# hongsukchoi/Pose2Mesh_RELEASE

Hardware: AMD Instinct MI355X
Metric: SMPL meshes/sec fwd+bwd at batch 256 (higher is better)
Workload: dtype f32 (emulated on the BF16 matrix pipe: every operand as 3 exact bf16 slices = 24-bit significands, 6 slice products per fp32 product, fp32 accumulate)

## Files before the change

### pose2mesh_release_amd/csrc/gemm.hip

```cpp
#include <cstdlib>
#include <type_traits>

#include "p2m_split.h"

namespace p2m {

constexpr int BM = 128;
constexpr int BK = 32;
constexpr int AS_LD = BK + 1;

struct GemmArgs {
  const float* A[3];
  const float* Bm;
  const float* bias;
  const float* addend;
  const float* act_scale;
  const float* act_shift;
  int act_relu;
  int pair_out;
  float* C[3];
  float* stats;
  long M;
  int nplanesA, Ka, a0_shift;
  int N, Nc;
// ... 359 lines not shown
    for (int ps = 0; ps < APASS; ps++) {
      int lf, lc;
      if (ROWS) {
        int i = rs_i0 + ps * AROWS + a_row;
        if (i >= g.nset) i = g.nset - 1;
        lf = g.ids[i];
        lc = g.compact ? i : lf;
      } else {
        long rf = m0 + ps * AROWS + a_row;
        if (rf >= g.M) rf = g.M - 1;
        lf = (int)(rf - m0);
        lc = lf;
      }
      voff0[ps] = (unsigned)(((lf >> g.a0_shift) * g.Ka + a_k4) * 4);
      voff12[ps] = (unsigned)((lc * g.Ka + a_k4) * 4);
    }
    const int b_nl = (pt >> 1) & 7;
    const int b_n = ((((pt % (BN * 2)) >> 1) >> 3) << 3) | ((b_nl & 3) << 1) | (b_nl >> 2), b_half = (pt & 1) * 8;
    const unsigned bx_voff = (unsigned)((((n0 + b_n) * 16) + b_half) * 2);
    const long bx_slice = (long)g.Npad * 16;

    f32x4 ra[NST][APASS];
    u32x4 rb[NST][NS];
    auto load_chunk = [&](int kc, f32x4 (&a)[APASS], u32x4 (&b)[NS]) {
      const int p = kc / cpp;
      const int k0 = (kc - p * cpp) * KB;
      const char* Ab = reinterpret_cast<const char*>(g.A[p] + (p == 0 ? sbase0 : sbase12) + k0);
#pragma unroll
      for (int ps = 0; ps < APASS; ps++)
#ifdef P2M_PL_ABL_NOLOAD
        a[ps] = f32x4{__uint_as_float(voff0[ps]), 1.f, 2.f, (float)(long)Ab};
#else
        a[ps] = *reinterpret_cast<const f32x4*>(Ab + (p == 0 ? voff0[ps] : voff12[ps]));
#endif
      const char* src0 = reinterpret_cast<const char*>(g.Bx + (long)((p * g.Ka + k0) >> 4) * (NS * bx_slice));
#pragma unroll
      for (int sl = 0; sl < NS; sl++) b[sl] = *reinterpret_cast<const u32x4*>(src0 + sl * 2 * bx_slice + bx_voff);
    };
    auto store_chunk = [&](int kc, f32x4 (&a)[APASS], const u32x4 (&b)[NS]) {
      const int buf = kc % NBUF;
      unsigned short* as = As + buf * A_BUF;
#pragma unroll
      for (int ps = 0; ps < APASS; ps++) asm volatile("" : "+v"(a[ps]));
      if (in_act && kc < cpp) {
        const f32x4 sc = *reinterpret_cast<const f32x4*>(&actco[kc * KB + a_k4]);
        const f32x4 sh = *reinterpret_cast<const f32x4*>(&actco[256 + kc * KB + a_k4]);
#pragma unroll
        for (int ps = 0; ps < APASS; ps++)
#pragma unroll
          for (int e = 0; e < 4; e++) a[ps][e] = fmaxf(fmaf(a[ps][e], sc[e], sh[e]), 0.f);
      }
#pragma unroll
      for (int ps = 0; ps < APASS; ps++) {
        u32x2 sl[NS];
#ifdef P2M_PL_ABL_NOSLICE
        for (int q = 0; q < NS; q++) sl[q] = u32x2{__float_as_uint(a[ps][q & 1]), __float_as_uint(a[ps][2 + (q & 1)])};
#else
        split_pack4<NS>(a[ps][0], a[ps][1], a[ps][2], a[ps][3], a_sc, sl);
#endif
        unsigned short* d = as + (ps * AROWS + a_row) * LDX + a_k4;
#pragma unroll
        for (int q = 0; q < NS; q++) *reinterpret_cast<u32x2*>(d + q * BM * LDX) = sl[q];
      }
      unsigned short* d = Bs + buf * B_BUF + b_n * LDX + b_half;
#pragma unroll
      for (int q = 0; q < NS; q++) *reinterpret_cast<u32x4*>(d + q * BN * LDX) = b[q];
    };
    const int last = n - 1;
#pragma unroll
    for (int i = 0; i < NST; i++) load_chunk(i < last ? i : last, ra[i], rb[i]);
#pragma unroll
    for (int i = 0; i < AHEAD; i++) {
      if (i < n) store_chunk(i, ra[i], rb[i]);
      load_chunk(NST + i < last ? NST + i : last, ra[i], rb[i]);
    }
    lds_barrier();
    int kc = 0;
    for (; kc + (NST - 1) + AHEAD + NST < n; kc += NST) {
#pragma unroll
      for (int i = 0; i < NST; i++) {
        store_chunk(kc + i + AHEAD, ra[(i + AHEAD) % NST], rb[(i + AHEAD) % NST]);
        load_chunk(kc + i + AHEAD + NST, ra[(i + AHEAD) % NST], rb[(i + AHEAD) % NST]);
        lds_barrier();
      }
    }
    for (; kc < n; kc += NST) {
#pragma unroll
      for (int i = 0; i < NST; i++) {
        if (kc + i < n) {
          if (kc + i + AHEAD < n) store_chunk(kc + i + AHEAD, ra[(i + AHEAD) % NST], rb[(i + AHEAD) % NST]);
          if (kc + i + AHEAD + NST < n) load_chunk(kc + i + AHEAD + NST, ra[(i + AHEAD) % NST], rb[(i + AHEAD) % NST]);
          lds_barrier();
        }
      }
    }
  } else {
    frag_t fa[NBUF - 1][NS][TM], fb[NBUF - 1][NS][TN];
    auto read_frags = [&](int kc, frag_t (&a)[NS][TM], frag_t (&b)[NS][TN]) {
      const int buf = kc % NBUF;
      const unsigned short* as = As + buf * A_BUF + (wm * 64 + l31) * LDX + lhi * 8;
      const unsigned short* bs = Bs + buf * B_BUF + (wn * WTN + l31) * LDX + lhi * 8;
#pragma unroll
      for (int sl = 0; sl < NS; sl++) {
#pragma unroll
        for (int i = 0; i < TM; i++)
          a[sl][i] = __builtin_bit_cast(frag_t, *reinterpret_cast<const u32x4*>(as + (sl * BM + i * 32) * LDX));
#pragma unroll
        for (int j = 0; j < TN; j++)
          b[sl][j] = __builtin_bit_cast(frag_t, *reinterpret_cast<const u32x4*>(bs + (sl * BN + j * 32) * LDX));
      }
    };
    auto mfmas = [&](const frag_t (&a)[NS][TM], const frag_t (&b)[NS][TN]) {
#define P2M_PAIR(SA, SB)                                                                       \
  _Pragma("unroll") for (int i = 0; i < TM; i++) _Pragma("unroll") for (int j = 0; j < TN; j++) \
      acc[i][j] = slice_mfma<NS>(a[SA][i], b[SB][j], acc[i][j]);
#ifdef P2M_PL_ABL_NOMFMA
      if constexpr (NS == 3) {
        P2M_PAIR(0, 0)
        for (int sl = 1; sl < NS; sl++)
          for (int i = 0; i < TM; i++) for (int j = 0; j < TN; j++) { asm volatile("" :: "v"(a[sl][i])); asm volatile("" :: "v"(b[sl][j])); }
      } else
#endif
      if constexpr (NS == 3) {
        P2M_PAIR(2, 0)
        P2M_PAIR(0, 2)
        P2M_PAIR(1, 1)
        P2M_PAIR(1, 0)
        P2M_PAIR(0, 1)
        P2M_PAIR(0, 0)
      } else {
        P2M_PAIR(1, 0)
        P2M_PAIR(0, 1)
        P2M_PAIR(0, 0)
      }
#undef P2M_PAIR
    };
    lds_barrier();
    for (int kc = 0; kc < n; kc++) {
      read_frags(kc, fa[0], fb[0]);
      mfmas(fa[0], fb[0]);
      lds_barrier();
    }
  }
  __syncthreads();
  if (!producer) {
    gemm_epilogue<BN, EXTRA, ROWS>(g, acc, smem, rowtab, mt, m0, n0, rs_i0, wm, wn, l31, lhi, descale);
  } else {
    if (g.stats != nullptr) {
      __syncthreads();
      __syncthreads();
      __syncthreads();
    }
  }
}

template <int NS>
__global__ void k_weight_split(const float* __restrict__ Bm, unsigned short* __restrict__ Bx, int K, int N, int Npad,
                               const unsigned* __restrict__ amax_in, int bits) {
  const long i = (long)blockIdx.x * blockDim.x + threadIdx.x;
  if (i >= (long)Npad * K) return;
  const int k = (int)(i / Npad), n = (int)(i - (long)k * Npad);
  const long sl = (long)Npad * 16;
  unsigned short* d = Bx + (long)(k >> 4) * NS * sl + (long)n * 16 + (k & 15);
  if constexpr (NS == 3) {
    unsigned h = 0, m = 0, l = 0;
    if (n < N) split3(Bm[(long)k * N + n], h, m, l);
    d[0] = (unsigned short)(h >> 16);
    d[sl] = (unsigned short)(m >> 16);
    d[2 * sl] = (unsigned short)(l >> 16);
  } else {
    unsigned* trailer = reinterpret_cast<unsigned*>(Bx + (long)NS * Npad * K);
    const unsigned word = *amax_in;
    if (i == 0 && amax_in != trailer) *trailer = word == 0u ? 0u : __float_as_uint(__builtin_ldexpf(__uint_as_float(word), bits));
    const float y = n < N ? Bm[(long)k * N + n] * exp2_int(slice_scale_exp(word, bits)) : 0.f;
    const _Float16 h = (_Float16)y;
    const _Float16 l = (_Float16)(y - (float)h);
    d[0] = __builtin_bit_cast(unsigned short, h);
    d[sl] = __builtin_bit_cast(unsigned short, l);
  }
}

__global__ __launch_bounds__(1024) void k_amax_one_block(const float* __restrict__ x, long n, unsigned* __restrict__ word) {
  __shared__ float red[16];
  float m = 0.f;
  const long n4 = (reinterpret_cast<uintptr_t>(x) & 15) == 0 ? n >> 2 : 0;
  const f32x4* x4 = reinterpret_cast<const f32x4*>(x);
  long i = threadIdx.x;
  for (; i + 7 * 1024 < n4; i += 8 * 1024) {
    f32x4 v[8];
#pragma unroll
    for (int u = 0; u < 8; u++) v[u] = x4[i + u * 1024];
#pragma unroll
    for (int u = 0; u < 8; u++)
      m = fmaxf(fmaxf(m, fmaxf(amax_abs(v[u][0]), amax_abs(v[u][1]))), fmaxf(amax_abs(v[u][2]), amax_abs(v[u][3])));
  }
  for (; i < n4; i += 1024) {
    const f32x4 v = x4[i];
    m = fmaxf(fmaxf(m, fmaxf(amax_abs(v[0]), amax_abs(v[1]))), fmaxf(amax_abs(v[2]), amax_abs(v[3])));
  }
  for (long j = n4 * 4 + threadIdx.x; j < n; j += 1024) m = fmaxf(m, amax_abs(x[j]));
#pragma unroll
  for (int o = 32; o > 0; o >>= 1) m = fmaxf(m, __shfl_xor(m, o));
  if ((threadIdx.x & 63) == 0) red[threadIdx.x >> 6] = m;
  __syncthreads();
  if (threadIdx.x == 0) {
    for (int w = 1; w < 16; w++) m = fmaxf(m, red[w]);
    *word = __float_as_uint(m);
  }
}
__device__ __forceinline__ void amax_commit_block(unsigned* word, float m) {
  __shared__ float wmax[4];
#pragma unroll
  for (int o = 32; o > 0; o >>= 1) m = fmaxf(m, __shfl_xor(m, o));
  if ((threadIdx.x & 63) == 0) wmax[threadIdx.x >> 6] = m;
  __syncthreads();
  if (threadIdx.x == 0) {
    m = fmaxf(fmaxf(wmax[0], wmax[1]), fmaxf(wmax[2], wmax[3]));
    if (m > 0.f) {
      const unsigned bits = __float_as_uint(m);
      if (bits > __hip_atomic_load(word, __ATOMIC_RELAXED, __HIP_MEMORY_SCOPE_AGENT)) atomicMax(word, bits);
    }
  }
}
__global__ __launch_bounds__(256) void k_amax(const float* __restrict__ x, int head, long n4, int tail,
                                              unsigned* __restrict__ word) {
  float m = 0.f;
  const f32x4* x4 = reinterpret_cast<const f32x4*>(x + head);
  const long stride = (long)gridDim.x * 256;
  long i = (long)blockIdx.x * 256 + threadIdx.x;
  for (; i + 3 * stride < n4; i += 4 * stride) {
    const f32x4 v0 = x4[i], v1 = x4[i + stride], v2 = x4[i + 2 * stride], v3 = x4[i + 3 * stride];
    auto mx = [](const f32x4& v) {
      return fmaxf(fmaxf(amax_abs(v[0]), amax_abs(v[1])), fmaxf(amax_abs(v[2]), amax_abs(v[3])));
    };
    m = fmaxf(m, fmaxf(fmaxf(mx(v0), mx(v1)), fmaxf(mx(v2), mx(v3))));
  }
  for (; i < n4; i += stride) {
    const f32x4 v = x4[i];
    m = fmaxf(fmaxf(m, fmaxf(amax_abs(v[0]), amax_abs(v[1]))), fmaxf(amax_abs(v[2]), amax_abs(v[3])));
  }
  if (blockIdx.x == 0) {
    if ((int)threadIdx.x < head) m = fmaxf(m, amax_abs(x[threadIdx.x]));
    if ((int)threadIdx.x < tail) m = fmaxf(m, amax_abs(x[head + n4 * 4 + threadIdx.x]));
  }
  amax_commit_block(word, m);
}
__global__ __launch_bounds__(256) void k_amax_rows(const float* __restrict__ x, RowSet rs, int B, int F,
                                                   unsigned* __restrict__ word) {
  const int f4 = F >> 2;
  const long tot = (long)B * rs.n * f4;
  float m = 0.f;
  for (long i = (long)blockIdx.x * 256 + threadIdx.x; i < tot; i += (long)gridDim.x * 256) {
    const long row = i / f4;
    const int c = (int)(i - row * f4);
    const int b = (int)(row / rs.n), r = (int)(row - (long)b * rs.n);
    const f32x4 v = *reinterpret_cast<const f32x4*>(x + ((long)b * rs.V + (rs.ids ? rs.ids[r] : r)) * F + c * 4);
    m = fmaxf(fmaxf(m, fmaxf(amax_abs(v[0]), amax_abs(v[1]))), fmaxf(amax_abs(v[2]), amax_abs(v[3])));
  }
  amax_commit_block(word, m);
}

__global__ void k_naive_gemm_planes(GemmArgs g) {
  long idx = (long)blockIdx.x * blockDim.x + threadIdx.x;
  if (idx >= g.M * g.N) return;
  long r = idx / g.N;
  int n = (int)(idx - r * g.N);
  float acc = 0.f;
  for (int p = 0; p < g.nplanesA; p++) {
    const float* a = g.A[p] + (r >> (p == 0 ? g.a0_shift : 0)) * g.Ka;
    const float* b = g.Bm + (long)p * g.Ka * g.N + n;
    for (int k = 0; k < g.Ka; k++) acc = fmaf(a[k], b[(long)k * g.N], acc);
  }
  if (g.bias) acc += g.bias[n];
  if (g.act_scale) acc = fmaf(acc, g.act_scale[n], g.act_shift[n]);
  if (g.act_relu) acc = fmaxf(acc, 0.f);
  if (g.addend) acc += g.addend[r * g.N + n];
  int q = n / g.Nc;
  g.C[q][r * g.Nc + (n - q * g.Nc)] = acc;
}

__global__ void k_naive_tile_stats(const float* __restrict__ Y, float* __restrict__ stats, long M, int N) {
  int tile = blockIdx.x;
  long r0 = (long)tile * BM;
  long r1 = r0 + BM < M ? r0 + BM : M;
  for (int n = threadIdx.x; n < N; n += blockDim.x) {
    float s = 0.f;
    for (long r = r0; r < r1; r++) s += Y[r * N + n];
    float mean = s / (float)(r1 - r0);
    float m2 = 0.f;
    for (long r = r0; r < r1; r++) {
      float d = Y[r * N + n] - mean;
      m2 += d * d;
    }
    stats[(long)tile * 2 * N + n] = s;
    stats[(long)tile * 2 * N + N + n] = m2;
  }
}

struct TnArgs {
  const float* A[3];
  const float* G[3];
  int Gc;
  float* P;
  float* Pdb;
  long M, chunk_rows;
  int nplanesA, Ka, a0_shift, Ktot, N;
// ... 677 lines not shown
      k = (int)(kk / Fin); fin = (int)(kk % Fin);
    } else if (layout == 2) {
      fout = (int)(idx / Fin);
      fin = (int)(idx - (long)fout * Fin);
    } else {
      long nn = idx % ((long)K * Fout);
      fin = (int)(idx / ((long)K * Fout));
      k = (int)(nn / Fout); fout = (int)(nn % Fout);
    }
    float t0 = 0.f, t1 = 0.f, t2 = 0.f, t3 = 0.f;
    int c = cg;
    for (; c + 3 * UNP_CG < nchunks; c += 4 * UNP_CG) {
      t0 += P[(long)c * tot + idx];
      t1 += P[(long)(c + UNP_CG) * tot + idx];
      t2 += P[(long)(c + 2 * UNP_CG) * tot + idx];
      t3 += P[(long)(c + 3 * UNP_CG) * tot + idx];
    }
    for (; c < nchunks; c += UNP_CG) t0 += P[(long)c * tot + idx];
    s = ((double)t0 + (double)t1) + ((double)t2 + (double)t3);
    if (P2 != nullptr) {
      const long o2 = (long)fin * Fout + fout, st2 = (long)Fin * Fout;
      float q0 = 0.f, q1 = 0.f;
      int c2 = cg;
      for (; c2 + UNP_CG < nchunks2; c2 += 2 * UNP_CG) {
        q0 += P2[(long)c2 * st2 + o2];
        q1 += P2[(long)(c2 + UNP_CG) * st2 + o2];
      }
      for (; c2 < nchunks2; c2 += UNP_CG) q0 += P2[(long)c2 * st2 + o2];
      s += ((double)q0 + (double)q1) * (k == 0 ? 1.0 : (k == 1 ? (double)fake_a : (double)fake_b));
    }
  }
  red[cg][e] = s;
  __syncthreads();
  if (cg == 0 && idx < tot) {
    double r = 0.0;
#pragma unroll
    for (int q = 0; q < UNP_CG; q++) r += red[q][e];
    const long o = (long)fout * Fin * K + (long)fin * K + k;
    dW[o] = accumulate ? dW[o] + (float)r : (float)r;
  }
  if (db != nullptr && Pdb != nullptr && (long)blockIdx.x * 32 < Fout) {
    __syncthreads();
    double r = 0.0;
    if (idx < Fout) {
      for (int c = cg; c < nchunks; c += UNP_CG) r += (double)Pdb[(long)c * pdb_stride + idx];
      if (Pdb2 != nullptr)
        for (int c2 = cg; c2 < nchunks2; c2 += UNP_CG) r += (double)Pdb2[(long)c2 * Fout + idx];
    }
    red[cg][e] = r;
    __syncthreads();
    if (cg == 0 && idx < Fout) {
      double t = 0.0;
#pragma unroll
      for (int q = 0; q < UNP_CG; q++) t += red[q][e];
      db[idx] = accumulate ? db[idx] + (float)t : (float)t;
    }
  }
}

}

using namespace p2m;

extern "C" int32_t p2m_stats_tile_rows(void) { return BM; }


static inline int slices_of(int arith) { return arith == P2M_ARITH_F16X2 ? 2 : 3; }
static inline const unsigned* weight_amax_word(const void* Bx, int arith, long Npad, long K) {
  return arith == P2M_ARITH_F16X2
             ? reinterpret_cast<const unsigned*>(static_cast<const unsigned short*>(Bx) + 2 * Npad * K)
             : nullptr;
}

extern "C" int64_t p2m_weight_split_elems(int32_t K, int32_t N, int32_t arith) {
  if (K <= 0 || N <= 0 || K % 16 != 0 || (arith != P2M_ARITH_BF16X3 && arith != P2M_ARITH_F16X2)) return 0;
  return (long)slices_of(arith) * (cdiv(N, 128) * 128ll) * K + (arith == P2M_ARITH_F16X2 ? 8 : 0);
}

extern "C" int p2m_weight_split(const float* Bm, int32_t K, int32_t N, int32_t arith, const void* amax_in,
                                int32_t amax_bits, void* Bx, void* stream) {
  P2M_CHECK_ARG(Bm && Bx && K > 0 && N > 0, "null pointer or empty shape");
  P2M_CHECK_ARG(K % 16 == 0, "K must be a multiple of 16");
  P2M_CHECK_ARG(arith == P2M_ARITH_BF16X3 || arith == P2M_ARITH_F16X2, "arith must be P2M_ARITH_BF16X3 or P2M_ARITH_F16X2");
  const int Npad = cdiv(N, 128) * 128;
  const dim3 grid(cdiv((long)Npad * K, 256));
  unsigned short* bx = static_cast<unsigned short*>(Bx);
  if (arith == P2M_ARITH_F16X2) {
    const unsigned* word = static_cast<const unsigned*>(amax_in);
    P2M_CHECK_ARG(amax_bits >= 0 && amax_bits <= 30, "amax_bits out of range");
    if (word == nullptr) {
      unsigned* trailer = const_cast<unsigned*>(weight_amax_word(Bx, arith, Npad, K));
      hipLaunchKernelGGL(k_amax_one_block, dim3(1), dim3(1024), 0, (hipStream_t)stream, Bm, (long)K * N, trailer);
      word = trailer;
      amax_bits = 0;
    }
    hipLaunchKernelGGL(k_weight_split<2>, grid, dim3(256), 0, (hipStream_t)stream, Bm, bx, K, N, Npad, word, amax_bits);
  } else {
    hipLaunchKernelGGL(k_weight_split<3>, grid, dim3(256), 0, (hipStream_t)stream, Bm, bx, K, N, Npad, nullptr, 0);
  }
  return check_launch("weight_split");
}

extern "C" int p2m_conv_weights_prepare(const p2m_conv_weights* dev_desc, int32_t n, int32_t arith, void* stream) {
  static_assert(sizeof(p2m_conv_weights) == sizeof(ConvWeights), "descriptor layout");
  P2M_CHECK_ARG(dev_desc != nullptr && n > 0, "null descriptor array or no layers");
  P2M_CHECK_ARG(arith == P2M_ARITH_BF16X3 || arith == P2M_ARITH_F16X2, "arith must be P2M_ARITH_BF16X3 or P2M_ARITH_F16X2");
  const ConvWeights* d = reinterpret_cast<const ConvWeights*>(dev_desc);
  hipStream_t s = (hipStream_t)stream;
  const dim3 grid(96, n);
  if (arith == P2M_ARITH_F16X2) {
    hipLaunchKernelGGL(k_conv_weights_amax, dim3(n), dim3(1024), 0, s, d);
    hipLaunchKernelGGL(k_conv_weights_images<2>, grid, dim3(256), 0, s, d);
  } else {
    hipLaunchKernelGGL(k_conv_weights_images<3>, grid, dim3(256), 0, s, d);
  }
  return check_launch("conv_weights_prepare");
}

extern "C" int p2m_amax(const float* x, int64_t n, void* word, void* stream) {
  P2M_CHECK_ARG(x && word && n >= 0, "null pointer");
  P2M_CHECK_ARG((reinterpret_cast<uintptr_t>(x) & 3) == 0, "x must be 4-byte aligned");
  if (n == 0) return P2M_OK;
  long head = (long)((16 - (reinterpret_cast<uintptr_t>(x) & 15)) & 15) / 4;
  if (head > n) head = n;
  const long n4 = (n - head) / 4;
  const int tail = (int)(n - head - 4 * n4);
  const int grid = (int)(n4 < 256l * 4 * 1024 ? (n4 > 0 ? cdiv(n4, 256 * 4) : 1) : 1024);
  hipLaunchKernelGGL(k_amax, dim3(grid), dim3(256), 0, (hipStream_t)stream, x, (int)head, n4, tail,
                     static_cast<unsigned*>(word));
  return check_launch("amax");
}

extern "C" int p2m_amax_rows(p2m_graph_t gh, int32_t row_set, const float* x, int32_t B, int32_t F, void* word,
                             void* stream) {
  P2M_CHECK_ARG(gh && x && word, "null pointer");
  P2M_CHECK_ARG(row_set >= 0 && row_set <= 4, "row_set must be 0 (live rows) or 1..4");
  P2M_CHECK_ARG(F > 0 && F % 4 == 0, "F must be a positive multiple of 4");
  const Graph& gr = *reinterpret_cast<const Graph*>(gh);
  RowSet rs;
  if (row_set == 0) {
    rs.V = gr.V;
    rs.ids = gr.live_ids;
    rs.n = gr.live_ids ? gr.n_live : gr.V;
  } else {
    rs = row_set_of(gr, row_set);
  }
  if (B <= 0 || rs.n == 0) return P2M_OK;
  const long tot = (long)B * rs.n * (F / 4);
  const int grid = (int)(tot < 256l * 2048 ? cdiv(tot, 256) : 2048);
  hipLaunchKernelGGL(k_amax_rows, dim3(grid), dim3(256), 0, (hipStream_t)stream, x, rs, B, F, static_cast<unsigned*>(word));
  return check_launch("amax_rows");
}

template <bool ROWS>
static void launch_gemm_planes(GemmArgs& g, bool extra, hipStream_t s) {
  const bool wide = (g.N % 128 == 0);
  g.ntn = wide ? g.N / 128 : cdiv(g.N, 64);
  const dim3 grid(cdiv(g.ntm, 8) * 8 * g.ntn);
  if (g.Bx != nullptr) {
#define P2M_LAUNCH_WS(BNv, EX)                                                                              \
  do {                                                                                                      \
    if (g.a_amax != nullptr) hipLaunchKernelGGL((k_gemm_planes_ws<BNv, EX, ROWS, 2>), grid, dim3(512), 0, s, g); \
    else hipLaunchKernelGGL((k_gemm_planes_ws<BNv, EX, ROWS, 3>), grid, dim3(512), 0, s, g);                 \
  } while (0)
    if (wide) { if (extra) P2M_LAUNCH_WS(128, true); else P2M_LAUNCH_WS(128, false); }
    else { if (extra) P2M_LAUNCH_WS(64, true); else P2M_LAUNCH_WS(64, false); }
#undef P2M_LAUNCH_WS
  } else {
#define P2M_LAUNCH(BNv, EX) hipLaunchKernelGGL((k_gemm_planes<BNv, 32, EX, ROWS>), grid, dim3(256), 0, s, g)
    if (wide) { if (extra) P2M_LAUNCH(128, true); else P2M_LAUNCH(128, false); }
    else { if (extra) P2M_LAUNCH(64, true); else P2M_LAUNCH(64, false); }
#undef P2M_LAUNCH
  }
}

extern "C" int p2m_gemm_planes(const float* A0, const float* A1, const float* A2, int32_t nplanesA, int32_t Ka,
                               int32_t a0_shift, const float* Bm, const void* Bsplit, int32_t arith,
                               const void* a_amax, int32_t a_bits, const float* bias,
                               const float* addend, float* C0, float* C1, float* C2, int32_t nplanesC, int32_t Nc,
                               int32_t pair_out, int64_t M, float* stats, const float* act_scale,
                               const float* act_shift, int32_t act_relu, void* amax_out, void* stream) {
  P2M_CHECK_ARG(nplanesA >= 1 && nplanesA <= 3 && nplanesC >= 1 && nplanesC <= 3, "plane count must be 1..3");
  P2M_CHECK_ARG(arith == P2M_ARITH_F32 || arith == P2M_ARITH_BF16X3 || arith == P2M_ARITH_F16X2, "unknown arithmetic");
  P2M_CHECK_ARG((act_scale == nullptr) == (act_shift == nullptr), "act_scale / act_shift must both be given or both NULL");
  P2M_CHECK_ARG(!((act_scale || act_relu) && (stats || pair_out)), "fused activation excludes stats and pair_out");
  P2M_CHECK_ARG(A0 && Bm && C0 && Ka > 0 && Nc > 0, "null pointer or empty shape");
  P2M_CHECK_ARG(a0_shift == 0 || a0_shift == 1, "a0_shift must be 0 or 1");
  if (M <= 0) return P2M_OK;
  GemmArgs g;
  g.A[0] = A0; g.A[1] = A1; g.A[2] = A2;
  g.C[0] = C0; g.C[1] = C1; g.C[2] = C2;
  for (int p = 0; p < nplanesA; p++) P2M_CHECK_ARG(g.A[p] != nullptr, "missing A plane");
  for (int p = 0; p < nplanesC; p++) P2M_CHECK_ARG(g.C[p] != nullptr, "missing C plane");
  P2M_CHECK_ARG((addend == nullptr && !pair_out) || nplanesC == 1, "addend / pair_out need a single output plane");
  P2M_CHECK_ARG(!(pair_out && stats), "pair_out and stats are mutually exclusive");
  g.Bm = Bm; g.bias = bias; g.addend = addend; g.pair_out = pair_out; g.stats = stats; g.M = M;
  g.act_scale = act_scale; g.act_shift = act_shift; g.act_relu = act_relu;
  g.nplanesA = nplanesA; g.Ka = Ka; g.a0_shift = a0_shift;
  g.N = nplanesC * Nc; g.Nc = Nc;
  g.ids = nullptr; g.nset = 0; g.V = 0; g.tps = 0; g.compact = 0; g.row_w = nullptr;
  g.Bx = nullptr; g.Npad = 0; g.Ktot = 0;
  g.a_amax = g.b_amax = nullptr; g.a_bits = 0;
  g.amax_out = static_cast<unsigned*>(amax_out);
  g.in_scale = g.in_shift = nullptr;
  hipStream_t s = (hipStream_t)stream;
  const bool mfma_ok = (Ka % BK == 0) && (g.N % 32 == 0) && (Nc % 32 == 0);
  if (!mfma_ok) {
    P2M_CHECK_ARG(!pair_out, "pair_out needs the MFMA path (Ka % 32 == 0, N % 32 == 0)");
    P2M_CHECK_ARG(!amax_out, "amax_out needs the MFMA path (Ka % 32 == 0, N % 32 == 0)");
    long tot = M * g.N;
    g.ntm = g.ntn = 0;
    hipLaunchKernelGGL(k_naive_gemm_planes, dim3(cdiv(tot, 256)), dim3(256), 0, s, g);
    if (stats) {
      P2M_CHECK_ARG(nplanesC == 1, "stats need a single output plane");
      hipLaunchKernelGGL(k_naive_tile_stats, dim3(cdiv(M, BM)), dim3(64), 0, s, C0, stats, (long)M, g.N);
    }
    return check_launch("gemm_planes(naive)");
  }
  if (arith != P2M_ARITH_F32) {
    P2M_CHECK_ARG(Bsplit != nullptr, "the slice arithmetics need the pre-split weight (p2m_weight_split)");
    P2M_CHECK_ARG(arith != P2M_ARITH_F16X2 || a_amax != nullptr, "P2M_ARITH_F16X2 needs the amax word of the A planes");
    g.Bx = static_cast<const unsigned short*>(Bsplit);
    g.Npad = cdiv(g.N, 128) * 128;
    g.Ktot = nplanesA * Ka;
    if (arith == P2M_ARITH_F16X2) {
      g.a_amax = static_cast<const unsigned*>(a_amax);
      g.a_bits = a_bits;
      g.b_amax = weight_amax_word(Bsplit, arith, g.Npad, g.Ktot);
    }
  }
  g.ntm = cdiv(M, BM);
  launch_gemm_planes<false>(g, addend != nullptr || pair_out, s);
  return check_launch("gemm_planes");
}

extern "C" int p2m_gemm_planes_rows(p2m_graph_t gh, int32_t row_set, int32_t B, const float* A0, const float* A1,
                                    const float* A2, int32_t nplanesA, int32_t Ka, int32_t a0_shift,
                                    int32_t planes_compact, const float* Bm, const void* Bsplit, int32_t arith,
                                    const void* a_amax, int32_t a_bits, const float* bias,
                                    const float* addend, float* C, int32_t N, float* stats, const float* act_scale,
                                    const float* act_shift, int32_t act_relu, void* amax_out, const float* in_scale,
                                    const float* in_shift, void* stream) {
  P2M_CHECK_ARG(gh && A0 && Bm && C, "null pointer");
  P2M_CHECK_ARG((in_scale == nullptr) == (in_shift == nullptr), "in_scale / in_shift must both be given or both NULL");
  P2M_CHECK_ARG(in_scale == nullptr || (arith != P2M_ARITH_F32 && Ka <= 256),
                "activation on load exists in the slice arithmetics only, for Ka <= 256");
  P2M_CHECK_ARG(arith == P2M_ARITH_F32 || arith == P2M_ARITH_BF16X3 || arith == P2M_ARITH_F16X2, "unknown arithmetic");
  P2M_CHECK_ARG(arith == P2M_ARITH_F32 || Bsplit != nullptr, "the slice arithmetics need the pre-split weight (p2m_weight_split)");
  P2M_CHECK_ARG(arith != P2M_ARITH_F16X2 || a_amax != nullptr, "P2M_ARITH_F16X2 needs the amax word of the A planes");
  P2M_CHECK_ARG((act_scale == nullptr) == (act_shift == nullptr), "act_scale / act_shift must both be given or both NULL");
  P2M_CHECK_ARG(!((act_scale || act_relu) && stats), "fused activation excludes stats");
  P2M_CHECK_ARG(row_set_valid(row_set), "row_set must be 1 (real), 2 (fake), 3 (paired real) or 4 (paired fake)");
  P2M_CHECK_ARG(nplanesA >= 1 && nplanesA <= 3, "plane count must be 1..3");
  P2M_CHECK_ARG(Ka > 0 && Ka % BK == 0 && N > 0 && N % 32 == 0, "Ka and N must be positive multiples of 32");
  P2M_CHECK_ARG(a0_shift == 0 || a0_shift == 1, "a0_shift must be 0 or 1");
  const Graph& gr = *reinterpret_cast<const Graph*>(gh);
  const RowSet rs = row_set_of(gr, row_set);
  if (B <= 0 || rs.n == 0) return P2M_OK;
  GemmArgs g;
  g.A[0] = A0; g.A[1] = A1; g.A[2] = A2;
  for (int p = 0; p < nplanesA; p++) P2M_CHECK_ARG(g.A[p] != nullptr, "missing A plane");
  g.C[0] = C; g.C[1] = nullptr; g.C[2] = nullptr;
  g.Bm = Bm; g.bias = bias; g.addend = addend; g.pair_out = 0; g.stats = stats;
  g.act_scale = act_scale; g.act_shift = act_shift; g.act_relu = act_relu;
  g.nplanesA = nplanesA; g.Ka = Ka; g.a0_shift = a0_shift; g.N = N; g.Nc = N;
  g.ids = rs.ids; g.nset = rs.n; g.V = rs.V; g.tps = cdiv(rs.n, BM); g.compact = planes_compact;
  g.row_w = (stats != nullptr && row_set == 2) ? gr.fake_wts : nullptr;
  g.Bx = arith == P2M_ARITH_F32 ? nullptr : static_cast<const unsigned short*>(Bsplit);
  g.Npad = cdiv(N, 128) * 128;
  g.Ktot = nplanesA * Ka;
  g.a_amax = g.b_amax = nullptr; g.a_bits = 0;
  if (arith == P2M_ARITH_F16X2) {
    g.a_amax = static_cast<const unsigned*>(a_amax);
    g.a_bits = a_bits;
    g.b_amax = weight_amax_word(Bsplit, arith, g.Npad, g.Ktot);
  }
  g.amax_out = static_cast<unsigned*>(amax_out);
  g.in_scale = in_scale; g.in_shift = in_shift;
  g.M = (long)B * g.tps * BM;
  g.ntm = B * g.tps;
  launch_gemm_planes<true>(g, addend != nullptr, (hipStream_t)stream);
  return check_launch("gemm_planes_rows");
}

extern "C" int32_t p2m_rows_tiles_per_sample(p2m_graph_t gh, int32_t row_set) {
  if (!gh || !row_set_valid(row_set)) return 0;
  const Graph& gr = *reinterpret_cast<const Graph*>(gh);
  return cdiv(row_set_of(gr, row_set).n, BM);
}

static int gemm_tn_impl(const float* A0, const float* A1, const float* A2, int32_t nplanesA, int32_t Ka,
                        int32_t a0_shift, const float* G0, const float* G1, const float* G2, int32_t nplanesG,
                        int32_t Gc, int64_t M, int64_t chunk_rows, float* P, float* Pdb, int32_t arith,
                        const void* a_amax, int32_t a_bits, const void* g_amax, int32_t g_bits, int32_t accumulate,
                        void* stream);
extern "C" int p2m_gemm_tn(const float* A0, const float* A1, const float* A2, int32_t nplanesA, int32_t Ka,
                           int32_t a0_shift, const float* G0, const float* G1, const float* G2, int32_t nplanesG,
                           int32_t Gc, int64_t M, int64_t chunk_rows, float* P, float* Pdb, int32_t arith,
                           const void* a_amax, int32_t a_bits, const void* g_amax, int32_t g_bits, void* stream) {
  return gemm_tn_impl(A0, A1, A2, nplanesA, Ka, a0_shift, G0, G1, G2, nplanesG, Gc, M, chunk_rows, P, Pdb, arith, a_amax,
                      a_bits, g_amax, g_bits, 0, stream);
}
extern "C" int p2m_gemm_tn_acc(const float* A, int32_t Ka, const float* G, int32_t N, int64_t M, float* P, int32_t arith,
                               const void* a_amax, const void* g_amax, void* stream) {
  const int64_t chunk_rows = ((M + 31) / 32) * 32;
  return gemm_tn_impl(A, nullptr, nullptr, 1, Ka, 0, G, nullptr, nullptr, 1, N, M, chunk_rows > 0 ? chunk_rows : 32, P,
                      nullptr, arith, a_amax, 0, g_amax, 0, 1, stream);
}
static int gemm_tn_impl(const float* A0, const float* A1, const float* A2, int32_t nplanesA, int32_t Ka,
                        int32_t a0_shift, const float* G0, const float* G1, const float* G2, int32_t nplanesG,
                        int32_t Gc, int64_t M, int64_t chunk_rows, float* P, float* Pdb, int32_t arith,
// ... 2 lines not shown
  P2M_CHECK_ARG(nplanesA >= 1 && nplanesA <= 3 && nplanesG >= 1 && nplanesG <= 3, "plane count must be 1..3");
  P2M_CHECK_ARG(arith == P2M_ARITH_F32 || arith == P2M_ARITH_BF16X3 || arith == P2M_ARITH_F16X2, "unknown arithmetic");
  P2M_CHECK_ARG(arith != P2M_ARITH_F16X2 || (a_amax && g_amax), "P2M_ARITH_F16X2 needs the amax words of both operands");
  const int N = nplanesG * Gc;
  P2M_CHECK_ARG(A0 && G0 && P && Ka > 0 && Gc > 0 && chunk_rows > 0, "null pointer or empty shape");
  P2M_CHECK_ARG(a0_shift == 0 || a0_shift == 1, "a0_shift must be 0 or 1");
  if (M <= 0) return P2M_OK;
  TnArgs g;
  g.A[0] = A0; g.A[1] = A1; g.A[2] = A2;
  for (int p = 0; p < nplanesA; p++) P2M_CHECK_ARG(g.A[p] != nullptr, "missing A plane");
  g.G[0] = G0; g.G[1] = G1; g.G[2] = G2; g.Gc = Gc;
  for (int p = 0; p < nplanesG; p++) P2M_CHECK_ARG(g.G[p] != nullptr, "missing G plane");
  g.P = P; g.Pdb = Pdb; g.M = M; g.chunk_rows = chunk_rows;
  g.nplanesA = nplanesA; g.Ka = Ka; g.a0_shift = a0_shift; g.Ktot = nplanesA * Ka; g.N = N;
  g.ids = nullptr; g.nset = 0; g.V = 0; g.splits = 1; g.compact = 0;
  g.a_amax = static_cast<const unsigned*>(a_amax); g.g_amax = static_cast<const unsigned*>(g_amax);
  g.a_bits = a_bits; g.g_bits = g_bits;
  g.a_scale = g.a_shift = nullptr;
  const int nchunks = cdiv(M, chunk_rows);
  g.nchunks = nchunks;
  g.accum = accumulate;
  P2M_CHECK_ARG(!accumulate || nchunks == 1, "accumulation needs the whole reduction in one chunk");
  hipStream_t s = (hipStream_t)stream;
  const bool mfma_ok = (Ka % 4 == 0) && (N % 32 == 0) && (Gc % 4 == 0) && (g.Ktot >= 32);
  if (!mfma_ok) {
    g.nkt = g.ntn = 0;
    int nout = g.Ktot * N;
    if (nout < N) nout = N;
    hipLaunchKernelGGL(k_naive_gemm_tn, dim3(cdiv(nout, 256), nchunks), dim3(256), 0, s, g);
    return check_launch("gemm_tn(naive)");
  }
  g.nkt = cdiv(g.Ktot, BM);
  const bool bx = arith != P2M_ARITH_F32;
  if (N % 128 == 0 || (bx && N > 128)) {
    g.ntn = cdiv(N, 128);
    const dim3 grid(g.nkt * g.ntn, nchunks), grid_ws((nchunks >= 8 ? cdiv(nchunks, 8) * 8 : nchunks) * g.nkt * g.ntn);
    if (arith == P2M_ARITH_F16X2) hipLaunchKernelGGL((k_gemm_tn_ws<128, false, 2>), grid_ws, dim3(512), 0, s, g);
    else if (bx) hipLaunchKernelGGL((k_gemm_tn_ws<128, false, 3>), grid_ws, dim3(512), 0, s, g);
    else hipLaunchKernelGGL((k_gemm_tn<128, false>), grid, dim3(256), 0, s, g);
  } else {
    g.ntn = cdiv(N, 64);
    const dim3 grid(g.nkt * g.ntn, nchunks), grid_ws((nchunks >= 8 ? cdiv(nchunks, 8) * 8 : nchunks) * g.nkt * g.ntn);
    if (arith == P2M_ARITH_F16X2) hipLaunchKernelGGL((k_gemm_tn_ws<64, false, 2>), grid_ws, dim3(512), 0, s, g);
    else if (bx) hipLaunchKernelGGL((k_gemm_tn_ws<64, false, 3>), grid_ws, dim3(512), 0, s, g);
    else hipLaunchKernelGGL((k_gemm_tn<64, false>), grid, dim3(256), 0, s, g);
  }
  return check_launch("gemm_tn");
}

extern "C" int p2m_gemm_tn_rows(p2m_graph_t gh, int32_t row_set, int32_t B, const float* A, int32_t Ka,
                                int32_t a0_shift, const float* G0, const float* G1, const float* G2, int32_t nplanesG,
                                int32_t Gc, int32_t planes_compact, int32_t splits, float* P, float* Pdb,
                                int32_t arith, const void* a_amax, const void* g_amax, int32_t g_bits,
                                const float* a_scale, const float* a_shift, void* stream) {
  P2M_CHECK_ARG(gh && A && G0 && P, "null pointer");
  P2M_CHECK_ARG((a_scale == nullptr) == (a_shift == nullptr), "a_scale / a_shift must both be given or both NULL");
  P2M_CHECK_ARG(a_scale == nullptr || arith != P2M_ARITH_F32, "activation on load exists in the slice arithmetics only");
  P2M_CHECK_ARG(arith == P2M_ARITH_F32 || arith == P2M_ARITH_BF16X3 || arith == P2M_ARITH_F16X2, "unknown arithmetic");
  P2M_CHECK_ARG(arith != P2M_ARITH_F16X2 || (a_amax && g_amax), "P2M_ARITH_F16X2 needs the amax words of both operands");
  P2M_CHECK_ARG(row_set_valid(row_set), "row_set must be 1 (real), 2 (fake), 3 (paired real) or 4 (paired fake)");
  P2M_CHECK_ARG(nplanesG >= 1 && nplanesG <= 3 && (splits >= 1 || splits <= -2),
                "plane count must be 1..3; splits >= 1, or <= -2 (that many whole samples per chunk)");
  P2M_CHECK_ARG(splits >= 1 || arith != P2M_ARITH_F32, "several samples per chunk exist in the slice arithmetics only");
  P2M_CHECK_ARG(Ka % 32 == 0 && Gc % 32 == 0, "Ka and Gc must be multiples of 32");
  P2M_CHECK_ARG(a0_shift == 0 || a0_shift == 1, "a0_shift must be 0 or 1");
  const Graph& gr = *reinterpret_cast<const Graph*>(gh);
  const RowSet rs = row_set_of(gr, row_set);
  if (B <= 0 || rs.n == 0) return P2M_OK;
  TnArgs g;
  g.A[0] = A; g.A[1] = nullptr; g.A[2] = nullptr;
  g.G[0] = G0; g.G[1] = G1; g.G[2] = G2; g.Gc = Gc;
  for (int p = 0; p < nplanesG; p++) P2M_CHECK_ARG(g.G[p] != nullptr, "missing G plane");
  const int N = nplanesG * Gc;
  g.P = P; g.Pdb = Pdb; g.M = (long)B * rs.n;
  const int spc = splits < 0 ? -splits : 1;
  if (splits < 0) splits = 1;
  g.chunk_rows = cdiv(rs.n, splits);
  g.nplanesA = 1; g.Ka = Ka; g.a0_shift = a0_shift; g.Ktot = Ka; g.N = N;
  g.ids = rs.ids; g.nset = rs.n; g.V = rs.V; g.splits = splits; g.compact = planes_compact;
  g.spc = spc; g.B = B;
  g.a_amax = static_cast<const unsigned*>(a_amax); g.g_amax = static_cast<const unsigned*>(g_amax);
  g.a_bits = 0; g.g_bits = g_bits;
  g.a_scale = a_scale; g.a_shift = a_shift;
  const int nchunks = spc > 1 ? cdiv(B, spc) : B * splits;
  g.nchunks = nchunks;
  hipStream_t s = (hipStream_t)stream;
  g.nkt = cdiv(g.Ktot, BM);
  const bool bx = arith != P2M_ARITH_F32;
  if (bx) g.chunk_rows = cdiv(g.chunk_rows, 16) * 16;
  if (N % 128 == 0 || (bx && N > 128)) {
    g.ntn = cdiv(N, 128);
    const dim3 grid(g.nkt * g.ntn, nchunks), grid_ws((nchunks >= 8 ? cdiv(nchunks, 8) * 8 : nchunks) * g.nkt * g.ntn);
    if (arith == P2M_ARITH_F16X2) hipLaunchKernelGGL((k_gemm_tn_ws<128, true, 2>), grid_ws, dim3(512), 0, s, g);
    else if (bx) hipLaunchKernelGGL((k_gemm_tn_ws<128, true, 3>), grid_ws, dim3(512), 0, s, g);
    else hipLaunchKernelGGL((k_gemm_tn<128, true>), grid, dim3(256), 0, s, g);
  } else {
    g.ntn = cdiv(N, 64);
    const dim3 grid(g.nkt * g.ntn, nchunks), grid_ws((nchunks >= 8 ? cdiv(nchunks, 8) * 8 : nchunks) * g.nkt * g.ntn);
    if (arith == P2M_ARITH_F16X2) hipLaunchKernelGGL((k_gemm_tn_ws<64, true, 2>), grid_ws, dim3(512), 0, s, g);
    else if (bx) hipLaunchKernelGGL((k_gemm_tn_ws<64, true, 3>), grid_ws, dim3(512), 0, s, g);
    else hipLaunchKernelGGL((k_gemm_tn<64, true>), grid, dim3(256), 0, s, g);
  }
  return check_launch("gemm_tn_rows");
}

extern "C" int p2m_weight_pack(const float* W, float* Wt, float* W2, float* W3, int32_t Fout, int32_t Fin, int32_t K,
                               void* stream) {
  P2M_CHECK_ARG(W && Wt && Fout > 0 && Fin > 0 && K > 0, "null pointer or empty shape");
  long tot = (long)Fout * Fin * K;
  if (K == 1 && W2 == nullptr && W3 == nullptr && (reinterpret_cast<uintptr_t>(W) & 15) == 0 &&
      (reinterpret_cast<uintptr_t>(Wt) & 15) == 0) {
    hipLaunchKernelGGL(k_transpose_tiled, dim3(cdiv(Fin, 64), cdiv(Fout, 64)), dim3(256), 0, (hipStream_t)stream, W, Wt, Fout,
                       Fin);
    return check_launch("weight_pack(transpose)");
  }
  hipLaunchKernelGGL(k_weight_pack, dim3(cdiv(tot, 256)), dim3(256), 0, (hipStream_t)stream, W, Wt, W2, W3, Fout, Fin, K);
  return check_launch("weight_pack");
}

extern "C" int p2m_weight_eff(const float* Wt, float* We, int32_t Ka, int32_t N, float a, float b, void* stream) {
  P2M_CHECK_ARG(Wt && We && Ka > 0 && N > 0, "null pointer or empty shape");
  hipLaunchKernelGGL(k_weight_eff, dim3(cdiv((long)Ka * N, 256)), dim3(256), 0, (hipStream_t)stream, Wt, We, Ka, N, a, b);
  return check_launch("weight_eff");
}

extern "C" int p2m_weight_grad_unpack2(const float* P, const float* Pdb, int32_t nchunks, const float* P2,
                                       const float* Pdb2, int32_t nchunks2, float s1, float s2, float* dW, float* db,
                                       int32_t Fout, int32_t Fin, int32_t K, int32_t accumulate, void* stream) {
  P2M_CHECK_ARG(P && P2 && dW && Fout > 0 && Fin > 0 && K == 3 && nchunks > 0 && nchunks2 > 0, "null pointer or bad shape");
  long tot = (long)Fout * Fin * K;
  hipLaunchKernelGGL(k_weight_grad_unpack, dim3(cdiv(tot, 32)), dim3(32 * UNP_CG), 0, (hipStream_t)stream, P, Pdb, nchunks,
                     dW, db, Fout, Fin, K, accumulate, 1, K * Fout, P2, Pdb2, nchunks2, s1, s2);
  return check_launch("weight_grad_unpack2");
}

extern "C" int p2m_weight_grad_unpack(const float* P, const float* Pdb, int32_t nchunks, float* dW, float* db,
                                      int32_t Fout, int32_t Fin, int32_t K, int32_t accumulate, int32_t layout,
                                      int32_t pdb_stride, void* stream) {
  P2M_CHECK_ARG(P && dW && Fout > 0 && Fin > 0 && K > 0 && nchunks > 0, "null pointer or empty shape");
  P2M_CHECK_ARG(layout >= 0 && layout <= 2 && (layout != 2 || K == 1), "layout must be 0, 1 or (K = 1 only) 2");
  long tot = (long)Fout * Fin * K;
  hipLaunchKernelGGL(k_weight_grad_unpack, dim3(cdiv(tot, 32)), dim3(32 * UNP_CG), 0, (hipStream_t)stream, P, Pdb, nchunks,
                     dW, db, Fout, Fin, K, accumulate, layout, pdb_stride, nullptr, nullptr, 0, 0.f, 0.f);
  return check_launch("weight_grad_unpack");
}

#ifdef P2M_TN_TRACE
extern "C" int p2m_tn_trace_dump(unsigned long long* out ) {
  if (hipDeviceSynchronize() != hipSuccess) return P2M_ERR_HIP;
  return hipMemcpyFromSymbol(out, HIP_SYMBOL(p2m::g_tn_tr), sizeof(unsigned long long) * 8 * 32 * 4) == hipSuccess ? P2M_OK
                                                                                                                : P2M_ERR_HIP;
}
#endif
```

Before: 6198.

## Add single-plane row-gather GEMM kernel with register-staged A passes for small K

Adds a new k_gemm_rows_k1 kernel for gathered-row GEMMs with one A plane, K up to 256 and presplit weights. All 256 threads load A rows into registers two passes ahead, then apply the optional input scale/shift+ReLU, split to bf16 slices and store to LDS. B fragments are double-buffered straight from global memory into registers. This replaces the warp-specialized 512-thread producer/consumer kernel on that path, aiming to cut its sync and producer overhead and to reach 2 blocks per CU via launch bounds. It is on by default through an environment toggle, and optional s_memtime tracing is included.

```diff
diff --git a/pose2mesh_release_amd/csrc/gemm.hip b/pose2mesh_release_amd/csrc/gemm.hip
--- a/pose2mesh_release_amd/csrc/gemm.hip
+++ b/pose2mesh_release_amd/csrc/gemm.hip
@@ -535,6 +535,206 @@
       __syncthreads();
     }
   }
+}
+
+#ifdef P2M_K1_TRACE
+__device__ unsigned long long g_k1_tr[4096][4];
+#define P2M_K1T(ev)                                                                      \
+  do {                                                                                   \
+    if (threadIdx.x == 0 && blockIdx.x < 4096) g_k1_tr[blockIdx.x][ev] = __builtin_amdgcn_s_memtime(); \
+  } while (0)
+#else
+#define P2M_K1T(ev) do { } while (0)
+#endif
+
+template <int BN, bool EXTRA, int NS, int KP>
+__global__ __launch_bounds__(256, 2) void k_gemm_rows_k1(GemmArgs g) {
+  typedef typename SliceFrag<NS>::type frag_t;
+  constexpr bool ROWS = true;
+  constexpr int WTN = BN / 2;
+  constexpr int TN = WTN / 32;
+  constexpr int TM = 2;
+  constexpr int LDX = KP + 8;
+  constexpr int TPR = KP / 4;
+  constexpr int RPS = 256 / TPR;
+  constexpr int NSW = BM / RPS;
+  constexpr int KSTEPS = KP / 16;
+  constexpr int A_IMG = NS * BM * LDX;
+  static_assert(KP == 64 || KP == 32, "pass width");
+  static_assert(A_IMG / 2 >= 2 * BN, "the epilogue's reduction buffer lives in the image");
+  __shared__ __attribute__((aligned(16))) float smem[A_IMG / 2 + ROWTAB_WORDS];
+  __shared__ __attribute__((aligned(16))) float actco[2 * 256];
+  unsigned short* As = reinterpret_cast<unsigned short*>(smem);
+  int* rowtab = reinterpret_cast<int*>(smem + A_IMG / 2);
+
+  int mt, nt;
+  if (!tile_of_block(blockIdx.x, g.ntm, g.ntn, mt, nt)) return;
+  P2M_K1T(0);
+  const int t = threadIdx.x;
+  const long m0 = (long)mt * BM;
+  const int n0 = nt * BN;
+  const int rs_b = mt / g.tps;
+  const int rs_i0 = (mt - rs_b * g.tps) * BM;
+  const int lane = t & 63, wave = t >> 6;
+  const int wm = wave >> 1, wn = wave & 1;
+  const int l31 = lane & 31, lhi = lane >> 5;
+  const int npass = g.Ka / KP;
+  const bool in_act = g.in_scale != nullptr;
+  const bool live = n0 + wn * WTN < g.N;
+  float a_sc = 1.f;
+  int descale = 0;
+  if (NS == 2) {
+    const int sa = slice_scale_exp(*g.a_amax, g.a_bits);
+    a_sc = exp2_int(sa);
+    descale = -(sa + slice_scale_exp(*g.b_amax, 0));
+  }
+
+  int rt_row = -1;
+  float rt_w = 0.f, co_sc = 0.f, co_sh = 0.f;
+  if (t < BM) {
+    const int i = rs_i0 + t;
+    if (i < g.nset) {
+      rt_row = rs_b * g.V + g.ids[i];
+      if (g.row_w != nullptr) rt_w = g.row_w[i];
+    }
+  }
+  if (in_act && t < g.Ka) {
+    co_sc = g.in_scale[t];
+    co_sh = g.in_shift[t];
+  }
+
+  const int a_g = t / TPR;
+  const int a_row = KP == 64 ? a_g : (((a_g & 1) << 2) | ((a_g >> 1) & 3) | ((a_g >> 3) << 3));
+  const int a_k4 = (t % TPR) * 4;
+  const long sbase0 = (((long)rs_b * g.V) >> g.a0_shift) * g.Ka;
+  unsigned voff[NSW];
+#pragma unroll
+  for (int ps = 0; ps < NSW; ps++) {
+    int i = rs_i0 + ps * RPS + a_row;
+    if (i >= g.nset) i = g.nset - 1;
+    voff[ps] = (unsigned)((((g.ids[i] >> g.a0_shift) * g.Ka) + a_k4) * 4);
+  }
+  f32x4 ra[2][NSW];
+  auto load_pass = [&](int p, f32x4 (&a)[NSW]) {
+    const char* Ab = reinterpret_cast<const char*>(g.A[0] + sbase0 + p * KP);
+#pragma unroll
+    for (int ps = 0; ps < NSW; ps++) a[ps] = *reinterpret_cast<const f32x4*>(Ab + voff[ps]);
+  };
+  auto store_pass = [&](int p, f32x4 (&a)[NSW]) {
+    if (in_act) {
+      const f32x4 sc = *reinterpret_cast<const f32x4*>(&actco[p * KP + a_k4]);
+      const f32x4 sh = *reinterpret_cast<const f32x4*>(&actco[256 + p * KP + a_k4]);
+#pragma unroll
+      for (int ps = 0; ps < NSW; ps++)
+#pragma unroll
+        for (int e = 0; e < 4; e++) a[ps][e] = fmaxf(fmaf(a[ps][e], sc[e], sh[e]), 0.f);
+    }
+#pragma unroll
+    for (int ps = 0; ps < NSW; ps++) {
+      u32x2 sl[NS];
+      split_pack4<NS>(a[ps][0], a[ps][1], a[ps][2], a[ps][3], a_sc, sl);
+      unsigned short* d = As + (ps * RPS + a_row) * LDX + a_k4;
+#pragma unroll
+      for (int q = 0; q < NS; q++) *reinterpret_cast<u32x2*>(d + q * BM * LDX) = sl[q];
+    }
+  };
+
+  load_pass(0, ra[0]);
+  if (npass > 1) load_pass(1, ra[1]);
+
+  const long bx_slice = (long)g.Npad * 16;
+  const int nsteps = g.Ka / 16;
+  unsigned bx_voff[TN];
+#pragma unroll
+  for (int j = 0; j < TN; j++) bx_voff[j] = (unsigned)((((n0 + wn * WTN + j * 32 + l31) * 16) + lhi * 8) * 2);
+  frag_t fb[2][NS][TN];
+  auto load_b = [&](int kc, frag_t (&b)[NS][TN]) {
+    const char* src0 = reinterpret_cast<const char*>(g.Bx + (long)kc * (NS * bx_slice));
+#pragma unroll
+    for (int sl = 0; sl < NS; sl++)
+#pragma unroll
+      for (int j = 0; j < TN; j++)
+        b[sl][j] = __builtin_bit_cast(frag_t, *reinterpret_cast<const u32x4*>(src0 + sl * 2 * bx_slice + bx_voff[j]));
+  };
+  if (live) load_b(0, fb[0]);
+
+  if (t < BM) {
+    rowtab[t] = rt_row;
+    if (g.row_w != nullptr) {
+      float* wtab = reinterpret_cast<float*>(rowtab + BM);
+      wtab[t] = rt_w;
+      float s = rt_w;
+#pragma unroll
+      for (int o = 32; o > 0; o >>= 1) s += __shfl_xor(s, o);
+      if ((t & 63) == 0) wtab[BM + (t >> 6)] = s;
+    }
+  }
+  if (in_act) {
+    if (t < g.Ka) {
+      actco[t] = co_sc;
+      actco[256 + t] = co_sh;
+    }
+    lds_block_barrier();
+  }
+
+  floatx16 acc[TM][TN];
+#pragma unroll
+  for (int i = 0; i < TM; i++)
+#pragma unroll
+    for (int j = 0; j < TN; j++)
+#pragma unroll
+      for (int r = 0; r < 16; r++) acc[i][j][r] = 0.f;
+
+  auto mfma_pass = [&](int p) {
+    const unsigned short* as = As + (wm * 64 + l31) * LDX + lhi * 8;
+#pragma unroll
+    for (int ks = 0; ks < KSTEPS; ks++) {
+      const int kc = p * KSTEPS + ks;
+      frag_t fa[NS][TM];
+#pragma unroll
+      for (int sl = 0; sl < NS; sl++)
+#pragma unroll
+        for (int i = 0; i < TM; i++)
+          fa[sl][i] = __builtin_bit_cast(frag_t, *reinterpret_cast<const u32x4*>(as + (sl * BM + i * 32) * LDX + ks * 16));
+      frag_t (&b)[NS][TN] = fb[ks & 1];
+      load_b(kc + 1 < nsteps ? kc + 1 : kc, fb[(ks + 1) & 1]);
+#define P2M_PAIR(SA, SB)                                                                       \
+  _Pragma("unroll") for (int i = 0; i < TM; i++) _Pragma("unroll") for (int j = 0; j < TN; j++) \
+      acc[i][j] = slice_mfma<NS>(fa[SA][i], b[SB][j], acc[i][j]);
+      if constexpr (NS == 3) {
+        P2M_PAIR(2, 0)
+        P2M_PAIR(0, 2)
+        P2M_PAIR(1, 1)
+        P2M_PAIR(1, 0)
+        P2M_PAIR(0, 1)
+        P2M_PAIR(0, 0)
+      } else {
+        P2M_PAIR(1, 0)
+        P2M_PAIR(0, 1)
+        P2M_PAIR(0, 0)
+      }
+#undef P2M_PAIR
+    }
+  };
+
+  for (int p = 0; p < npass; p += 2) {
+#pragma unroll
+    for (int h = 0; h < 2; h++) {
+      const int pp = p + h;
+      if (pp < npass) {
+        if (pp > 0) lds_block_barrier();
+        store_pass(pp, ra[h]);
+        if (pp + 2 < npass) load_pass(pp + 2, ra[h]);
+        lds_block_barrier();
+        if (pp == 0) P2M_K1T(1);
+        if (live) mfma_pass(pp);
+      }
+    }
+  }
+  P2M_K1T(2);
+  __syncthreads();
+  gemm_epilogue<BN, EXTRA, ROWS>(g, acc, smem, rowtab, mt, m0, n0, rs_i0, wm, wn, l31, lhi, descale);
+  P2M_K1T(3);
 }
 
 template <int NS>
@@ -1518,11 +1718,32 @@
   return check_launch("amax_rows");
 }
 
+static bool rows_k1() {
+  static const bool v = [] { const char* e = getenv("P2M_ROWS_K1"); return e ? atoi(e) != 0 : true; }();
+  return v;
+}
+
 template <bool ROWS>
 static void launch_gemm_planes(GemmArgs& g, bool extra, hipStream_t s) {
   const bool wide = (g.N % 128 == 0);
   g.ntn = wide ? g.N / 128 : cdiv(g.N, 64);
   const dim3 grid(cdiv(g.ntm, 8) * 8 * g.ntn);
+  if constexpr (ROWS) {
+    if (g.nplanesA == 1 && g.Ka <= 256 && g.Bx != nullptr && rows_k1()) {
+#define P2M_LAUNCH_K1(BNv, EX, KPv)                                                                          \
+  do {                                                                                                      \
+    if (g.a_amax != nullptr) hipLaunchKernelGGL((k_gemm_rows_k1<BNv, EX, 2, KPv>), grid, dim3(256), 0, s, g); \
+    else hipLaunchKernelGGL((k_gemm_rows_k1<BNv, EX, 3, KPv>), grid, dim3(256), 0, s, g);                    \
+  } while (0)
+#define P2M_LAUNCH_K1_KP(BNv, EX) \
+  do { if (g.Ka % 64 == 0) P2M_LAUNCH_K1(BNv, EX, 64); else P2M_LAUNCH_K1(BNv, EX, 32); } while (0)
+      if (wide) { if (extra) P2M_LAUNCH_K1_KP(128, true); else P2M_LAUNCH_K1_KP(128, false); }
+      else { if (extra) P2M_LAUNCH_K1_KP(64, true); else P2M_LAUNCH_K1_KP(64, false); }
+#undef P2M_LAUNCH_K1_KP
+#undef P2M_LAUNCH_K1
+      return;
+    }
+  }
   if (g.Bx != nullptr) {
 #define P2M_LAUNCH_WS(BNv, EX)                                                                              \
   do {                                                                                                      \
@@ -1831,3 +2052,10 @@
                                                                                                                 : P2M_ERR_HIP;
 }
 #endif
+#ifdef P2M_K1_TRACE
+extern "C" int p2m_k1_trace_dump(unsigned long long* out ) {
+  if (hipDeviceSynchronize() != hipSuccess) return P2M_ERR_HIP;
+  return hipMemcpyFromSymbol(out, HIP_SYMBOL(p2m::g_k1_tr), sizeof(unsigned long long) * 4096 * 4) == hipSuccess ? P2M_OK
+                                                                                                                : P2M_ERR_HIP;
+}
+#endif
```

Result: faster. 6276 (median of 6 runs) (+1.3%).
